# mcx/AgileRL

Measured on AMD Instinct MI355X. Metric: population env-steps/sec + learner updates/sec, 8-agent PPO at 1/2/4/8 MI355X, higher is better.
Workload: dtype f32 (GAE carry f64); 1 GPU; config 2: one 8-agent PPO population sharded 8 agents per GPU, 128 vec envs per agent, T=16, batch 128, 4 epochs, MLP enc[64]->64 + heads[64] (shared encoder), tournament every 5 iterations; population=8, pop_per_gpu=8, num_envs=128, learn_step=2048, batch_size=128, update_epochs=4, learner=fused, parallelism=population-sharded x1

## Files before the change

### agilerl_amd/csrc/learner.hip

```cpp
#include <cmath>
#include <cstdlib>
#include <type_traits>

#include "agx_common.h"
#include "rollout.h"

namespace agx {

#ifndef AGX_LEARN_UNIFORM
#define AGX_LEARN_UNIFORM 1
#endif
#ifndef AGX_LEARN_RS2
#define AGX_LEARN_RS2 0
#endif

constexpr int kNT = 512;
constexpr int kNW = kNT / kWave;
constexpr int kSB = 32;
constexpr int kMaxSlot = 10;
constexpr int kMaxK = 16;
constexpr int kMaxPT = 32;
constexpr int kMaxA = 16;
constexpr int kMaxBlk = 28;

typedef unsigned v4u __attribute__((ext_vector_type(4)));

struct NetDims {
    int D, A, ne, eo[3], ha, hc;
};

struct Blk {
    int f0, len, rowlen, l0, ldst;
};

struct LearnPlan {
    int ok;
    int D, A, ne, ein[3], eout[3], eaff[3], lat, ha, hc, H, n;
    int f_ew[3], f_eb[3], f_eg[3], f_ebe[3];
    int f_aw, f_ab, f_ag, f_abe, f_aow, f_aob, f_cw, f_cb, f_cg, f_cbe, f_cow, f_cob;
    int l_ew[3], l_eld[3], l_eb[3], l_eg[3], l_ebe[3];
    int l_hw, l_hld, l_hb, l_hg, l_hbe;
    int l_aow, l_aold, l_aob, l_cow, l_cold, l_cob;
    int param_end;
    int l_x0, ld_x0, l_xe[3], ld_xe[3], l_re[3], l_xh, ld_xh, l_rh;
    int l_s1, l_s2, ld_s;
    int l_lg, l_dlg, l_dvb, l_val, l_row;
    int l_red, red_e[3], red_h, l_stat, l_stamp;
    int l_grad;
    int lds_floats, act_floats;
    int slab;
    int nt[6], ncol[6], slot0[6], nslot[6], nslots;
    int nblk;
    Blk blk[kMaxBlk];
};

constexpr int rup(int x, int m) { return (x + m - 1) / m * m; }

constexpr LearnPlan make_plan(NetDims d) {
    LearnPlan pl{};
    pl.ok = 0;
    pl.D = d.D;
    pl.A = d.A;
    pl.ne = d.ne;
    if (pl.ne < 2 || pl.ne > 3 || pl.A < 1 || pl.A > kMaxA || pl.D < 1 || pl.D > 128) return pl;
    int prev = pl.D;
    for (int e = 0; e < pl.ne; ++e) {
        pl.ein[e] = prev;
        pl.eout[e] = d.eo[e];
        pl.eaff[e] = e < pl.ne - 1;
        if (pl.eout[e] % 16 || pl.eout[e] > 128 || pl.eout[e] < 16) return pl;
        prev = pl.eout[e];
    }
    pl.lat = prev;
    pl.ha = d.ha;
    pl.hc = d.hc;
    pl.H = pl.ha + pl.hc;
    if (pl.ha % 16 || pl.hc % 16 || pl.ha < 16 || pl.hc < 16 || pl.H > 128) return pl;
    int f = 0;
    for (int e = 0; e < pl.ne; ++e) {
        pl.f_ew[e] = f;
// ... 46 lines not shown
    pl.l_x0 = off; off += rup(kSB * pl.ld_x0, 4);
    for (int e = 0; e < pl.ne; ++e) {
        pl.ld_xe[e] = pl.eout[e] + 2;
        pl.l_xe[e] = off; off += kSB * pl.ld_xe[e];
        pl.l_re[e] = off; off += 2 * kSB;
    }
    pl.ld_xh = pl.H + 2;
    pl.l_xh = off; off += kSB * pl.ld_xh;
    pl.l_rh = off; off += 2 * kSB;
    int wmax = pl.H;
    for (int e = 0; e < pl.ne; ++e) wmax = wmax > pl.eout[e] ? wmax : pl.eout[e];
    pl.ld_s = wmax + 2;
    pl.l_s1 = off; off += kSB * pl.ld_s;
    pl.l_s2 = off; off += kSB * pl.ld_s;
    pl.l_lg = off; off += kSB * kMaxA;
    pl.l_val = off; off += kSB;
    pl.act_floats = off;
    pl.l_dlg = off; off += kSB * kMaxA;
    pl.l_dvb = off; off += kSB * kMaxA;
    pl.l_row = off; off += 6 * kSB;
    pl.l_grad = pl.l_x0;
    if (off - pl.l_x0 < pl.param_end) off = pl.l_x0 + pl.param_end;
    int red = 0;
    for (int e = 0; e < pl.ne; ++e) {
        pl.red_e[e] = red;
        red += (pl.eaff[e] ? 3 : 1) * kNW * pl.eout[e];
    }
    pl.red_h = red;
    red += 3 * kNW * pl.H;
    pl.l_red = off; off += red;
    pl.l_stat = off; off += 5 * kNW;
    off = rup(off, 2);
    pl.l_stamp = off; off += 2 * 80;
    pl.lds_floats = off;
    if (pl.lds_floats * 4 > 160 * 1024) return pl;
    pl.slab = rup(pl.param_end + 4 + 2 * kNW * kMaxK, 64);
    int slot = 0;
    for (int g = 0; g < pl.ne + 3; ++g) {
        int fo = 0, fi = 0;
        if (g < pl.ne) { fo = pl.eout[g]; fi = pl.ein[g]; }
        else if (g == pl.ne) { fo = pl.H; fi = pl.lat; }
        else if (g == pl.ne + 1) { fo = 16; fi = pl.ha + 1; }
        else { fo = 16; fi = pl.hc + 1; }
        pl.ncol[g] = (fi + 15) / 16;
        pl.nt[g] = (fo / 16) * pl.ncol[g];
        pl.slot0[g] = slot;
        pl.nslot[g] = (pl.nt[g] + kNW - 1) / kNW;
        slot += pl.nslot[g];
    }
    pl.nslots = slot;
    if (slot > kMaxSlot) return pl;
    int nb = 0;
    auto blk = [&](int f0, int len, int rowlen, int l0, int ldst) {
        if (len > 0) pl.blk[nb++] = Blk{f0, len, rowlen, l0, ldst};
    };
    for (int e = 0; e < pl.ne; ++e) {
        const int fo = pl.eout[e], fi = pl.ein[e];
        blk(pl.f_ew[e], fo * fi, fi, pl.l_ew[e], pl.l_eld[e]);
        blk(pl.f_eb[e], fo, fo, pl.l_eb[e], fo);
        if (pl.eaff[e]) {
            blk(pl.f_eg[e], fo, fo, pl.l_eg[e], fo);
            blk(pl.f_ebe[e], fo, fo, pl.l_ebe[e], fo);
        }
    }
    blk(pl.f_aw, pl.ha * pl.lat, pl.lat, pl.l_hw, pl.l_hld);
    blk(pl.f_ab, pl.ha, pl.ha, pl.l_hb, pl.ha);
// ... 499 lines not shown
            asm volatile("s_getreg_b32 %0, hwreg(HW_REG_XCC_ID)" : "=s"(x));
            __hip_atomic_store(xc + kk, (unsigned)(x & 15) + 1u, __ATOMIC_RELAXED, __HIP_MEMORY_SCOPE_AGENT);
            asm volatile("s_waitcnt vmcnt(0)" ::: "memory");
            unsigned *ctr = g.cnt + 2 * g.P + 1 + p;
            __hip_atomic_fetch_add(ctr, 1u, __ATOMIC_RELAXED, __HIP_MEMORY_SCOPE_AGENT);
            unsigned spins = 0;
            int ok = 1;
            while (__hip_atomic_load(ctr, __ATOMIC_RELAXED, __HIP_MEMORY_SCOPE_AGENT) < (unsigned)g.K) {
                __builtin_amdgcn_s_sleep(1);
                if (++spins > kSpinMax) {
                    __hip_atomic_store(tmo_v, 1u, __ATOMIC_RELAXED, __HIP_MEMORY_SCOPE_AGENT);
                    if (err_v) __hip_atomic_fetch_or(err_v, 1u, __ATOMIC_RELAXED, __HIP_MEMORY_SCOPE_AGENT);
                    ok = 0;
                    break;
                }
            }
            stat[4 * kNW] = ok ? 1.f : 0.f;
        }
        __syncthreads();
        if (stat[4 * kNW] == 0.f) return;
        const int ln = vlane();
        const unsigned v = ln < g.K ? __hip_atomic_load(xc + ln, __ATOMIC_RELAXED, __HIP_MEMORY_SCOPE_AGENT) : 0u;
        const unsigned v0 = __builtin_amdgcn_readlane(v, 0);
        bool same = v0 != 0u;
        for (int q = 1; q < g.K; ++q) same = same && __builtin_amdgcn_readlane(v, q) == v0;
        local = same && !g.write_through;
    }

    float *slab_p = in_vgpr(g.slabs + (g.K > 1 ? (size_t)p * 2 * g.K * pl.slab : 0));
    float *sum_p = in_vgpr(g.sums + (g.K > 1 ? (size_t)p * 2 * pl.slab : 0));
    unsigned *ctr1 = in_vgpr(g.cnt + p);
    unsigned *ctr2 = in_vgpr(g.cnt + g.P + 1 + p);
    unsigned *ctr3 = in_vgpr(g.cnt + 3 * g.P + 1 + (size_t)g.P * kMaxK + p);
    for (int e = 0; e < Ep; ++e) {
        for (int mb = 0; mb < nmb; ++mb) {
            const long long s0 = (long long)mb * Bp;
            const int bsz = (int)((s0 + Bp <= S) ? Bp : S - s0);
            const float inv_b = 1.f / (float)bsz;
            const int tid = vtid();
            f4 acc[kMaxSlot];
#pragma unroll
            for (int s = 0; s < kMaxSlot; ++s) acc[s] = f4{0.f, 0.f, 0.f, 0.f};
            for (int i = tid; i < pl.l_stat - pl.l_red; i += kNT) sm[pl.l_red + i] = 0.f;
            float lsum = 0.f, klsum = 0.f;
            const int upd = e * nmb + mb;
            float *base = g.K > 1 ? to_sgpr(slab_p + (size_t)(upd & 1) * g.K * pl.slab) : nullptr;
            const auto slab_rsrc = __builtin_amdgcn_make_buffer_rsrc(base + (size_t)kk * pl.slab, 0,
                                                                     __builtin_amdgcn_readfirstlane(pl.slab * 4),
                                                                     0x00020000);
            auto emit_tiles = [&](auto gc, auto fn) {
                constexpr int gg = decltype(gc)::value;
                AGX_IDS;
#pragma unroll
                for (int j = 0; j < pl.nslot[gg]; ++j) {
                    const int t = wave + kNW * j;
                    if (t < pl.nt[gg]) {
                        const int o0 = (t / pl.ncol[gg]) * 16, i0 = (t % pl.ncol[gg]) * 16;
                        const int col = i0 + lr16;
#pragma unroll
                        for (int i = 0; i < 4; ++i) {
                            const int o = o0 + lq * 4 + i;
                            const float x = acc[pl.slot0[gg] + j][i];
                            if constexpr (gg < pl.ne) {
                                if (col < pl.ein[gg]) fn(pl.l_ew[gg] + o * pl.l_eld[gg] + col, x);
                            } else if constexpr (gg == pl.ne) {
                                fn(pl.l_hw + o * pl.l_hld + col, x);
                            } else if constexpr (gg == pl.ne + 1) {
                                if (o < pl.A) {
                                    if (col < pl.ha) fn(pl.l_aow + o * pl.l_aold + col, x);
                                    else if (col == pl.ha) fn(pl.l_aob + o, x);
                                }
                            } else {
                                if (o == 0) {
                                    if (col < pl.hc) fn(pl.l_cow + col, x);
                                    else if (col == pl.hc) fn(pl.l_cob, x);
                                }
                            }
                        }
                    }
                }
            };
            auto put_l = [&](int l, float x) {
                __builtin_amdgcn_raw_buffer_store_b32(__builtin_bit_cast(unsigned, x), slab_rsrc, l * 4, 0, 0);
            };
            auto put_w = [&](int l, float x) {
                __builtin_amdgcn_raw_buffer_store_b32(__builtin_bit_cast(unsigned, x), slab_rsrc, l * 4, 0, 16);
            };
            auto slab_put = [&](int l, float x) {
                if (local) put_l(l, x);
                else put_w(l, x);
            };
            auto emit_slab = [&](auto gc) {
                if (local) emit_tiles(gc, put_l);
                else emit_tiles(gc, put_w);
            };
            const auto sum_rsrc = __builtin_amdgcn_make_buffer_rsrc(
                g.K > 1 ? to_sgpr(sum_p + (size_t)(upd & 1) * pl.slab) : nullptr, 0,
                __builtin_amdgcn_readfirstlane(pl.slab * 4), 0x00020000);
            auto partner_sync = [&](unsigned *ctr, unsigned target, int st0, int st1) -> bool {
                asm volatile("s_waitcnt vmcnt(0)" ::: "memory");
                __syncthreads();
                const int tid = vtid();
                if (tid == 0) {
                    const unsigned before = __hip_atomic_fetch_add(ctr, 1u, __ATOMIC_RELAXED, __HIP_MEMORY_SCOPE_AGENT);
                    AGX_STAMP(st0);
                    unsigned spins = 0;
                    int ok = 1;
                    while (before + 1u < target &&
                           __hip_atomic_load(ctr, __ATOMIC_RELAXED, __HIP_MEMORY_SCOPE_AGENT) < target) {
                        __builtin_amdgcn_s_sleep(1);
                        if (++spins > kSpinMax) {
                            __hip_atomic_store(tmo_v, 1u, __ATOMIC_RELAXED, __HIP_MEMORY_SCOPE_AGENT);
                            if (err_v) __hip_atomic_fetch_or(err_v, 1u, __ATOMIC_RELAXED, __HIP_MEMORY_SCOPE_AGENT);
                            ok = 0;
                            break;
                        }
                    }
                    asm volatile("s_waitcnt vmcnt(0)" ::: "memory");
                    stat[4 * kNW] = ok ? 1.f : 0.f;
                    AGX_STAMP(st1);
                }
                __syncthreads();
                return stat[4 * kNW] != 0.f;
            };
            const bool direct = g.K > 1;

            for (int sb = kk * SB; sb < bsz; sb += g.K * SB) {
                const bool last_sb = sb + g.K * SB >= bsz;
                const int nrow = bsz - sb < SB ? bsz - sb : SB;
                const int jsb = (sb / SB) / g.K;
                const int stb = jsb < 4 ? jsb * 16 : 80;
                const int tid = vtid();
                AGX_STAMP(stb + 0);
                {
                    auto commit = [&](const Pre &x) {
                        __builtin_amdgcn_s_waitcnt(0x0F70);
#pragma unroll
                        for (int k = 0; k < kPreObs; ++k) {
                            const int i = tid + k * kNT;
                            if (i < SB * pl.D) sm[pl.l_x0 + (i / pl.D) * pl.ld_x0 + i % pl.D] = i < nrow * pl.D ? x.ob[k] : 0.f;
                        }
                        constexpr int npad = pl.ld_x0 - pl.D;
#pragma unroll
                        for (int k = 0; k < (SB * npad + kNT - 1) / kNT; ++k) {
                            const int i = tid + k * kNT;
                            if (i < SB * npad) sm[pl.l_x0 + (i / npad) * pl.ld_x0 + pl.D + i % npad] = 0.f;
                        }
                        if (tid < 4 * kSB) rowf[tid] = tid % kSB < nrow ? __builtin_bit_cast(float, x.rv) : 0.f;
                        else if (tid < 5 * kSB) acts[tid - 4 * kSB] = tid - 4 * kSB < nrow ? (int)x.rv : 0;
                        else if (tid < 6 * kSB) legal[tid - 5 * kSB] = (has_mask && tid - 5 * kSB < nrow) ? x.rv : 0xffffffffu;
                    };
                    if constexpr (!kPrefetch) {
                        commit(fetch(e, mb, sb));
                    } else {
                        if (pre.e != e || pre.mb != mb || pre.sb != sb) pre = fetch(e, mb, sb);
                        commit(pre);
                        AGX_STAMP(stb + 4);
                        int ne = e, nm = mb, ns = sb + g.K * SB;
// ... 148 lines not shown
                            c2 += dxh[i] * xh[i];
                        }
                    }
                    const float rs0 = rl ? r0 : 0.f, rs1 = rl ? r1 : 0.f;
                    const float ma1 = rsum(a1) * (1.f / (float)F0), ma2 = rsum(a2) * (1.f / (float)F0);
                    const float mc1 = rsum(c1) * (1.f / (float)F1), mc2 = rsum(c2) * (1.f / (float)F1);
                    float *rd = sm + pl.l_red + pl.red_h;
                    float cs[3][NC];
#pragma unroll
                    for (int i = 0; i < NC; ++i) {
                        const int j = sub + W * i;
                        const bool g0 = W * i < split;
                        const float dz = (g0 ? rs0 : rs1) * (dxh[i] - (g0 ? ma1 : mc1) - xh[i] * (g0 ? ma2 : mc2));
                        if (rl) sm[pl.l_s2 + r * pl.ld_s + j] = dz;
                        cs[0][i] = rl ? dz : 0.f;
                        cs[1][i] = dyp[i] * xh[i];
                        cs[2][i] = dyp[i];
                    }
                    if constexpr (W == 16) {
#pragma unroll
                        for (int k = 0; k < 3; ++k)
#pragma unroll
                            for (int i = 0; i < NC; ++i) cs[k][i] += swz16(cs[k][i]);
                    }
                    if constexpr (W == 32 || (W == 16 && SB > 16)) {
#pragma unroll
                        for (int k = 0; k < 3; ++k)
#pragma unroll
                            for (int i = 0; i < NC; ++i)
                                cs[k][i] += __builtin_bit_cast(
                                    float, __builtin_amdgcn_ds_bpermute((lane ^ 32) << 2, __builtin_bit_cast(int, cs[k][i])));
                    }
                    if (lane < W) {
#pragma unroll
                        for (int k = 0; k < 3; ++k) {
                            float o[NC];
#pragma unroll
                            for (int i = 0; i < NC; ++i) o[i] = rd[(k * kNW + wave) * F + sub + W * i];
#pragma unroll
                            for (int i = 0; i < NC; ++i) rd[(k * kNW + wave) * F + sub + W * i] = o[i] + cs[k][i];
                        }
                    }
                }
                __syncthreads();
                AGX_STAMP(stb + 3);

                auto ln_bwd = [&](auto Fc, auto dybc, auto ldyc, auto xbc, auto ldxc, auto rbc, auto gbc, auto bbc,
                                  auto redc, auto affc) {
                    constexpr int F = decltype(Fc)::value;
                    constexpr int dyb = decltype(dybc)::value, ldy = decltype(ldyc)::value;
                    constexpr int xb = decltype(xbc)::value, ldx = decltype(ldxc)::value;
                    constexpr int rb = decltype(rbc)::value, gb = decltype(gbc)::value, bb = decltype(bbc)::value;
                    constexpr int red = decltype(redc)::value;
                    constexpr bool aff = decltype(affc)::value;
                    constexpr int W = (SB == 8 && F % 64 == 0) ? 64 : ((SB <= 16 && F % 32 == 0) ? 32 : 16);
                    constexpr int NC = F / W;
                    const int lane = vlane(), wave = swave();
                    const int sub = lane & (W - 1);
                    const int r = wrow<W>(lane, wave);
                    const bool rl = r < SB;
                    float xh[NC], dxh[NC], dyp[NC];
                    float a1 = 0.f, a2 = 0.f;
                    const float rs0 = rl ? sm[rb + 2 * r] : 0.f;
#pragma unroll
                    for (int i = 0; i < NC; ++i) {
                        const int j = sub + W * i;
                        const float dy = rl ? sm[dyb + r * ldy + j] : 0.f;
                        xh[i] = rl ? sm[xb + r * ldx + j] : 0.f;
                        const float gam = aff ? sm[gb + j] : 1.f;
                        const float y = aff ? xh[i] * gam + sm[bb + j] : xh[i];
                        dyp[i] = y > 0.f ? dy : 0.f;
                        dxh[i] = dyp[i] * gam;
                        a1 += dxh[i];
                        a2 += dxh[i] * xh[i];
                    }
                    const float ma1 = wrow_sum<W>(a1) * (1.f / (float)F), ma2 = wrow_sum<W>(a2) * (1.f / (float)F);
                    float *rd = sm + pl.l_red + red;
                    constexpr int NV = aff ? 3 : 1;
                    float cs[NV][NC];
#pragma unroll
                    for (int i = 0; i < NC; ++i) {
                        const int j = sub + W * i;
                        const float dz = rs0 * (dxh[i] - ma1 - xh[i] * ma2);
                        if (rl) sm[pl.l_s2 + r * pl.ld_s + j] = dz;
                        cs[0][i] = rl ? dz : 0.f;
                        if constexpr (aff) {
                            cs[1][i] = dyp[i] * xh[i];
                            cs[2][i] = dyp[i];
                        }
                    }
                    if constexpr (W == 16) {
#pragma unroll
                        for (int k = 0; k < NV; ++k)
#pragma unroll
                            for (int i = 0; i < NC; ++i)
                                cs[k][i] += __builtin_bit_cast(
                                    float, __builtin_amdgcn_ds_swizzle(__builtin_bit_cast(int, cs[k][i]), 0x401f));
                    }
                    if constexpr (W == 32 || (W == 16 && SB > 16)) {
#pragma unroll
                        for (int k = 0; k < NV; ++k)
#pragma unroll
                            for (int i = 0; i < NC; ++i)
                                cs[k][i] += __builtin_bit_cast(
                                    float, __builtin_amdgcn_ds_bpermute((lane ^ 32) << 2, __builtin_bit_cast(int, cs[k][i])));
                    }
                    if (lane < W) {
#pragma unroll
                        for (int k = 0; k < NV; ++k) {
                            float o[NC];
#pragma unroll
                            for (int i = 0; i < NC; ++i) o[i] = rd[(k * kNW + wave) * F + sub + W * i];
#pragma unroll
                            for (int i = 0; i < NC; ++i) rd[(k * kNW + wave) * F + sub + W * i] = o[i] + cs[k][i];
                        }
                    }
                };
                {
                    AGX_IDS;
                    constexpr int ga = pl.ne + 1, gc = pl.ne + 2;
#pragma unroll
                    for (int j = 0; j < pl.nslot[ga]; ++j) {
                        const int t = wave + kNW * j;
                        if (t < pl.nt[ga]) {
                            const int i0 = (t % pl.ncol[ga]) * 16;
                            acc[pl.slot0[ga] + j] = mfma_tile<SB>(
                                acc[pl.slot0[ga] + j], [&](int m, int k) { return sm[pl.l_dlg + k * kMaxA + m]; },
                                [&](int k, int n) {
                                    const int c = i0 + n;
                                    const float x = sm[pl.l_s1 + k * pl.ld_s + (c < pl.ha ? c : pl.ha - 1)];
                                    return x * (c < pl.ha ? 1.f : 0.f) + (c == pl.ha ? 1.f : 0.f);
                                });
                        }
                    }
#pragma unroll
                    for (int j = 0; j < pl.nslot[gc]; ++j) {
                        const int t = wave + kNW * j;
                        if (t < pl.nt[gc]) {
                            const int i0 = (t % pl.ncol[gc]) * 16;
                            acc[pl.slot0[gc] + j] = mfma_tile<SB>(
                                acc[pl.slot0[gc] + j], [&](int m, int k) { return sm[pl.l_dvb + k * kMaxA + m]; },
                                [&](int k, int n) {
                                    const int c = i0 + n;
                                    const float x = sm[pl.l_s1 + k * pl.ld_s + pl.ha + (c < pl.hc ? c : pl.hc - 1)];
                                    return x * (c < pl.hc ? 1.f : 0.f) + (c == pl.hc ? 1.f : 0.f);
                                });
                        }
// ... 9 lines not shown
                        if (t < pl.nt[gh]) {
                            const int o0 = (t / pl.ncol[gh]) * 16, i0 = (t % pl.ncol[gh]) * 16;
                            acc[pl.slot0[gh] + j] = mfma_tile<SB>(
                                acc[pl.slot0[gh] + j], [&](int m, int k) { return sm[pl.l_s2 + k * pl.ld_s + o0 + m]; },
                                [&](int k, int n) { return relu(sm[pl.l_xe[Le] + k * pl.ld_xe[Le] + i0 + n]); });
                        }
                    }
                    if (direct && last_sb) emit_slab(IC(gh));
                    constexpr int MT = m_tiles<SB>();
                    constexpr int nt = MT * (pl.lat / 16);
                    for (int t = wave; t < nt; t += kNW) {
                        const int m0 = (t % MT) * 16, n0 = (t / MT) * 16;
                        f4 c = f4{0.f, 0.f, 0.f, 0.f};
                        c = mfma_tile<pl.H>(c, [&](int m, int k) { return sm[pl.l_s2 + (m0 + m) * pl.ld_s + k]; },
                                            [&](int k, int n) { return sm[pl.l_hw + k * pl.l_hld + n0 + n]; });
                        if (SB >= 16 || lq * 4 < SB) {
#pragma unroll
                            for (int i = 0; i < 4; ++i) sm[pl.l_xh + (m0 + lq * 4 + i) * pl.ld_xh + n0 + lr16] = c[i];
                        }
                    }
                }
                __syncthreads();
                AGX_STAMP(stb + 6);

                auto enc_bwd = [&](auto Lc) {
                    constexpr int L = decltype(Lc)::value;
                    constexpr int fin = pl.ein[L], fout = pl.eout[L];
                    AGX_IDS;
                    constexpr int dyb = L == pl.ne - 1 ? pl.l_xh : pl.l_s1;
                    constexpr int ldy = L == pl.ne - 1 ? pl.ld_xh : pl.ld_s;
                    ln_bwd(IC(fout), IC(dyb), IC(ldy), IC(pl.l_xe[L]), IC(pl.ld_xe[L]), IC(pl.l_re[L]), IC(pl.l_eg[L]),
                           IC(pl.l_ebe[L]), IC(pl.red_e[L]), BC(pl.eaff[L] != 0));
                    __syncthreads();
                    constexpr bool in_aff = L > 0 && pl.eaff[L > 0 ? L - 1 : 0];
                    constexpr int xb = L == 0 ? pl.l_x0 : pl.l_xe[L > 0 ? L - 1 : 0];
                    constexpr int ldx = L == 0 ? pl.ld_x0 : pl.ld_xe[L > 0 ? L - 1 : 0];
                    constexpr int gbase = L > 0 ? pl.l_eg[L > 0 ? L - 1 : 0] : 0;
                    constexpr int bbase = L > 0 ? pl.l_ebe[L > 0 ? L - 1 : 0] : 0;
#pragma unroll
                    for (int j = 0; j < pl.nslot[L]; ++j) {
                        const int t = wave + kNW * j;
                        if (t < pl.nt[L]) {
                            const int o0 = (t / pl.ncol[L]) * 16, i0 = (t % pl.ncol[L]) * 16;
                            const int col = i0 + lr16;
                            const bool cv = col < fin;
                            const float gam = (in_aff && cv) ? sm[gbase + col] : 1.f;
                            const float bet = (in_aff && cv) ? sm[bbase + col] : 0.f;
                            acc[pl.slot0[L] + j] = mfma_tile<SB>(
                                acc[pl.slot0[L] + j], [&](int m, int k) { return sm[pl.l_s2 + k * pl.ld_s + o0 + m]; },
                                [&](int k, int n) {
                                    const float x = sm[xb + k * ldx + i0 + n];
                                    if constexpr (L == 0) return x;
                                    else return cv ? relu(x * gam + bet) : 0.f;
                                });
                        }
                    }
                    if (direct && last_sb) emit_slab(IC(L));
                    if constexpr (L > 0) {
                        constexpr int MT = m_tiles<SB>();
                        constexpr int nt = MT * (fin / 16);
                        for (int t = wave; t < nt; t += kNW) {
                            const int m0 = (t % MT) * 16, n0 = (t / MT) * 16;
                            f4 c = f4{0.f, 0.f, 0.f, 0.f};
                            c = mfma_tile<fout>(c, [&](int m, int k) { return sm[pl.l_s2 + (m0 + m) * pl.ld_s + k]; },
                                                [&](int k, int n) { return sm[pl.l_ew[L] + k * pl.l_eld[L] + n0 + n]; });
                            if (SB >= 16 || lq * 4 < SB) {
#pragma unroll
                                for (int i = 0; i < 4; ++i) sm[pl.l_s1 + (m0 + lq * 4 + i) * pl.ld_s + n0 + lr16] = c[i];
                            }
                        }
                    }
                    __syncthreads();
                };
                if constexpr (pl.ne == 3) enc_bwd(IC(2));
                enc_bwd(IC(1));
                enc_bwd(IC(0));
                AGX_STAMP(stb + 7);
            }

            float *G = sm + pl.l_grad;
            auto gput = [&](int l, float x) { G[l] = x; };
            if (!direct) {
                emit_tiles(IC(0), gput);
                emit_tiles(IC(1), gput);
                if constexpr (pl.ne == 3) emit_tiles(IC(2), gput);
                emit_tiles(IC(pl.ne), gput);
                emit_tiles(IC(pl.ne + 1), gput);
                emit_tiles(IC(pl.ne + 2), gput);
            } else if (kk * SB >= bsz) {
                emit_slab(IC(0));
                emit_slab(IC(1));
                if constexpr (pl.ne == 3) emit_slab(IC(2));
                emit_slab(IC(pl.ne));
                emit_slab(IC(pl.ne + 1));
                emit_slab(IC(pl.ne + 2));
            }
            auto vdump = [&](auto Lc, auto put) {
                constexpr int L = decltype(Lc)::value;
                constexpr int F = L < pl.ne ? pl.eout[L < pl.ne ? L : 0] : pl.H;
                constexpr int nv = (L < pl.ne && !pl.eaff[L < pl.ne ? L : 0]) ? 1 : 3;
                constexpr int red = L < pl.ne ? pl.red_e[L < pl.ne ? L : 0] : pl.red_h;
                const int tid = vtid();
#pragma unroll
                for (int rnd = 0; rnd < (nv * F + kNT - 1) / kNT; ++rnd) {
                    const int idx = tid + rnd * kNT;
                    if (idx >= nv * F) break;
                    const int k = idx / F, j = idx % F;
                    float pv[kNW];
#pragma unroll
                    for (int w = 0; w < kNW; ++w) pv[w] = sm[pl.l_red + red + (k * kNW + w) * F + j];
                    float x = 0.f;
#pragma unroll
                    for (int w = 0; w < kNW; ++w) x += pv[w];
                    int l;
                    if constexpr (L < pl.ne) {
                        l = (k == 0 ? pl.l_eb[L < pl.ne ? L : 0] : (k == 1 ? pl.l_eg[L < pl.ne ? L : 0] : pl.l_ebe[L < pl.ne ? L : 0])) + j;
                    } else {
                        l = (k == 0 ? pl.l_hb : (k == 1 ? pl.l_hg : pl.l_hbe)) + j;
                    }
                    put(l, x);
                }
            };
            auto vdump_all = [&](auto put) {
                vdump(IC(0), put);
                vdump(IC(1), put);
                if constexpr (pl.ne == 3) vdump(IC(2), put);
                vdump(IC(pl.ne), put);
            };
            if (!direct) vdump_all(gput);
            else if (local) vdump_all(put_l);
            else vdump_all(put_w);
            AGX_STAMP(64 + 9);
            __syncthreads();
            float lmb = lsum, klmb = klsum;
            {
                AGX_IDS;
                block_sum2(lmb, klmb, stat, 2, lane, wave);
            }
            float gr[kMaxPT];
            constexpr int NQ = (2 * kNW * KM + 63) / 64;
            float vq[NQ];
            if (g.K > 1) {
                if (tid == 0) {
                    slab_put(pl.param_end, lmb);
                    slab_put(pl.param_end + 1, klmb);
                }
                if (!partner_sync(ctr1, (unsigned)(g.K * (upd + 1)), 64 + 11, 64 + 12)) return;
                {
                    const int tid = vtid();
                    const auto rs = __builtin_amdgcn_make_buffer_rsrc(
                        base, 0, __builtin_amdgcn_readfirstlane(g.K * pl.slab * 4), 0x00020000);
                    bool rs_done = false;
#if AGX_LEARN_RS2
                    if constexpr (JN == 1) {
                        if (oc1 - oc0 <= kNT / 2) {
                            constexpr int KH = KM / 2;
                            const int h = tid >= kNT / 2 ? 1 : 0;
                            const int c = oc0 + (tid & (kNT / 2 - 1));
                            const int cl = c < oc1 ? c : oc0;
                            f4 x[KH];
#pragma unroll
                            for (int q = 0; q < KH; ++q) {
                                const int qq = KH * h + q, qs = qq < g.K ? qq : g.K - 1;
                                const f4 v = __builtin_bit_cast(
                                    f4, __builtin_amdgcn_raw_buffer_load_b128(rs, (qs * pl.slab + 4 * cl) * 4, 0, 16));
                                x[q] = qq < g.K ? v : f4{0.f, 0.f, 0.f, 0.f};
                            }
                            f4 t = x[0];
#pragma unroll
                            for (int q = 1; q < KH; ++q) t += x[q];
                            f4 *xch = reinterpret_cast<f4 *>(sm + pl.l_x0);
                            if (h) xch[tid - kNT / 2] = t;
                            __syncthreads();
                            if (!h) {
                                t += xch[tid];
                                if (c == n4) {
                                    if (local) __builtin_amdgcn_raw_buffer_store_b128(__builtin_bit_cast(v4u, t), sum_rsrc, c * 16, 0, 0);
                                    else __builtin_amdgcn_raw_buffer_store_b128(__builtin_bit_cast(v4u, t), sum_rsrc, c * 16, 0, 16);
                                }
                            }
#pragma unroll
                            for (int cc = 0; cc < 4; ++cc) gr[cc] = (!h && c < pc1) ? t[cc] : 0.f;
                            rs_done = true;
                        }
                    }
#endif
#pragma unroll
                    for (int j = 0; j < kUsed4; ++j) {
                        if (rs_done) break;
                        const int c = oc0 + tid + kNT * j;
                        f4 t = f4{0.f, 0.f, 0.f, 0.f};
                        if (j >= jn_own) {
#pragma unroll
                            for (int cc = 0; cc < 4; ++cc) gr[4 * j + cc] = 0.f;
                            continue;
                        }
                        if (c < oc1) {
                            f4 x[KM];
#pragma unroll
                            for (int q = 0; q < KM; ++q)
                                x[q] = q < g.K ? __builtin_bit_cast(f4, __builtin_amdgcn_raw_buffer_load_b128(
                                                                           rs, (q * pl.slab + 4 * c) * 4, 0, 16))
                                               : f4{0.f, 0.f, 0.f, 0.f};
                            t = x[0];
#pragma unroll
                            for (int q = 1; q < KM; ++q)
                                if (q < g.K) t += x[q];
                            if (c == n4) {
                                if (local) __builtin_amdgcn_raw_buffer_store_b128(__builtin_bit_cast(v4u, t), sum_rsrc, c * 16, 0, 0);
                                else __builtin_amdgcn_raw_buffer_store_b128(__builtin_bit_cast(v4u, t), sum_rsrc, c * 16, 0, 16);
                            }
                        }
#pragma unroll
                        for (int cc = 0; cc < 4; ++cc) gr[4 * j + cc] = c < pc1 ? t[cc] : 0.f;
                    }
                    AGX_STAMP(64 + 3);
                    float n0 = 0.f, n1 = 0.f;
#pragma unroll
                    for (int i = 0; i < 4 * kUsed4; ++i) {
                        if ((i >> 2) >= jn_own) break;
                        const bool valid = (vbits >> i) & 1u, crit = (gbits >> i) & 1u;
                        gr[i] = valid ? gr[i] : 0.f;
                        const float x2 = gr[i] * gr[i];
                        n1 += crit ? x2 : 0.f;
                        n0 += crit ? 0.f : x2;
                    }
                    const int lane = vlane(), wave = swave();
                    const float r0 = row_sum(n0), r1 = row_sum(n1);
                    const float w0 = readlane_f(r0, 0) + readlane_f(r0, 16) + readlane_f(r0, 32) + readlane_f(r0, 48);
                    const float w1 = readlane_f(r1, 0) + readlane_f(r1, 16) + readlane_f(r1, 32) + readlane_f(r1, 48);
                    if (lane < 2) {
                        const float w = lane ? w1 : w0;
                        const int o = (pl.param_end + 4 + (kk * kNW + wave) * 2 + lane) * 4;
                        if (local) __builtin_amdgcn_raw_buffer_store_b32(__builtin_bit_cast(unsigned, w), sum_rsrc, o, 0, 0);
                        else __builtin_amdgcn_raw_buffer_store_b32(__builtin_bit_cast(unsigned, w), sum_rsrc, o, 0, 16);
                    }
                }
                AGX_STAMP(64 + 13);
                if (!partner_sync(ctr2, (unsigned)(g.K * (upd + 1)), 64 + 8, 64 + 15)) return;
                {
                    const int lane = vlane();
                    const int np = 2 * kNW * g.K;
#pragma unroll
                    for (int q = 0; q < NQ; ++q) {
                        const float x = __builtin_bit_cast(
                            float, __builtin_amdgcn_raw_buffer_load_b32(sum_rsrc, (pl.param_end + 4 + 64 * q + lane) * 4, 0, 16));
                        vq[q] = lane + 64 * q < np ? x : 0.f;
                    }
                }
                const unsigned lw = __builtin_amdgcn_raw_buffer_load_b32(sum_rsrc, pl.param_end * 4, 0, 16);
                const unsigned kw = __builtin_amdgcn_raw_buffer_load_b32(sum_rsrc, (pl.param_end + 1) * 4, 0, 16);
                lmb = __builtin_bit_cast(float, __builtin_amdgcn_readfirstlane(lw));
                klmb = __builtin_bit_cast(float, __builtin_amdgcn_readfirstlane(kw));
            }

            float t0 = 0.f, t1 = 0.f;
            if (!direct) {
                const f4 *G4 = reinterpret_cast<const f4 *>(G);
#pragma unroll
                for (int j = 0; j < kUsed4; ++j) {
                    const int c = own_c(j);
                    const f4 x = c < pc1 ? G4[c] : f4{0.f, 0.f, 0.f, 0.f};
#pragma unroll
                    for (int cc = 0; cc < 4; ++cc) gr[4 * j + cc] = x[cc];
                }
                float n0 = 0.f, n1 = 0.f;
#pragma unroll
                for (int i = 0; i < 4 * kUsed4; ++i) {
                    const bool valid = (vbits >> i) & 1u, crit = (gbits >> i) & 1u;
                    gr[i] = valid ? gr[i] : 0.f;
                    const float x2 = gr[i] * gr[i];
                    n1 += crit ? x2 : 0.f;
                    n0 += crit ? 0.f : x2;
                }
                AGX_IDS;
                {
                    const float r0 = row_sum(n0), r1 = row_sum(n1);
                    const float w0 = readlane_f(r0, 0) + readlane_f(r0, 16) + readlane_f(r0, 32) + readlane_f(r0, 48);
                    const float w1 = readlane_f(r1, 0) + readlane_f(r1, 16) + readlane_f(r1, 32) + readlane_f(r1, 48);
                    if (lane == 0) {
                        stat[wave] = w0;
                        stat[kNW + wave] = w1;
                    }
                }
                __syncthreads();
                for (int i = 0; i < kNW; ++i) {
// ... 125 lines not shown
        const int l = 4 * own_c(i >> 2) + (i & 3);
        if ((vbits >> i) & 1u) {
            int grp;
            const int f = lds_to_flat<C>(l, grp);
            gp[f] = sm[l];
            gm[f] = am[i];
            gv[f] = av[i];
        }
    }
    if constexpr (ST)
        if (g.stamps && b == 0 && tid < 80) g.stamps[tid] = reinterpret_cast<const long long *>(sm + pl.l_stamp)[tid];
    if (tid == 0 && kk == 0) {
        if (loss_out_v) loss_out_v[p] = loss_total / ((float)S * (float)Ep);
        if (kl_out_v) kl_out_v[p] = n_done ? (float)(kl_total / (double)n_done) : 0.f;
        if (epochs_out_v) epochs_out_v[p] = epochs_done;
        *step_v = step0 + n_done;
    }
#undef IC
#undef BC
}

__global__ void ppo_gather_kernel(const float *__restrict__ obs, const long long *__restrict__ act,
                                  const float *__restrict__ old_logp, const float *__restrict__ adv,
                                  const float *__restrict__ ret, const float *__restrict__ old_v,
                                  const double *__restrict__ adv_stats, const long long *__restrict__ perms,
                                  const unsigned char *__restrict__ masks, int A,
                                  long long S, int D, int P, float *__restrict__ gobs, int *__restrict__ gact,
                                  unsigned *__restrict__ gmask, float *__restrict__ grow,
                                  unsigned *__restrict__ counters, int ncounters, const int *__restrict__ epochs_p,
                                  unsigned *__restrict__ err) {
    const int ep = blockIdx.y;
    const int p = ep % P;
    const long long j = (long long)blockIdx.x * blockDim.x + threadIdx.x;
    if (blockIdx.x == 0 && blockIdx.y == 0)
        for (int i = threadIdx.x; i < ncounters; i += blockDim.x) counters[i] = 0u;
    if (j >= S) return;
    if (epochs_p && ep / P >= epochs_p[p]) return;
    long long src = perms[(size_t)ep * S + j];
    if (src < 0 || src >= S) {
        if (err) __hip_atomic_fetch_or(err, AGX_LEARN_ERR_PERM, __ATOMIC_RELAXED, __HIP_MEMORY_SCOPE_AGENT);
        src = 0;
    }
    const size_t sp = (size_t)p * S + src;
    for (int d = 0; d < D; ++d) gobs[((size_t)ep * S + j) * D + d] = obs[sp * D + d];
    gact[(size_t)ep * S + j] = (int)act[sp];
    if (masks) {
        unsigned bits = 0;
        for (int a = 0; a < A; ++a) bits |= (masks[sp * A + a] != 0 ? 1u : 0u) << a;
        gmask[(size_t)ep * S + j] = bits;
    }
    float *gr = grow + (size_t)ep * 4 * S;
    double a = adv[sp];
    if (adv_stats) a = (a - adv_stats[2 * p]) * (1.0 / (adv_stats[2 * p + 1] + 1e-8));
    gr[j] = old_logp[sp];
    gr[S + j] = (float)a;
    gr[2 * S + j] = ret[sp];
    gr[3 * S + j] = old_v[sp];
}

template <class C>
__device__ __forceinline__ void act_body(const ActArgs &g, float *sm, bool resident, long long *st = nullptr) {
    constexpr LearnPlan pl = C::plan;
    const int p = blockIdx.y, n0 = blockIdx.x * kSB;
    const int tid = threadIdx.x, lane = tid & 63, wave = tid >> 6;
    const int nrow = g.N - n0 < kSB ? g.N - n0 : kSB;
    const float *ob = g.obs + (size_t)p * g.obs_pstride + (size_t)n0 * pl.D;
    constexpr int kObsIt = (kSB * pl.D + kNT - 1) / kNT;
    float obv[kObsIt];
// ... 246 lines not shown
    return (size_t)L.plan->lds_floats * sizeof(float);
}

static int max_partners(int64_t P) {
    int k = kMaxK;
    if (const char *e = getenv("AGX_LEARN_SPLIT")) k = atoi(e);
    if (k < 1) k = 1;
    if (k > kMaxK) k = kMaxK;
    const int64_t fit = cu_count() / (P > 0 ? P : 1);
    if (fit < k) k = fit < 1 ? 1 : (int)fit;
    return k;
}
static void pick_split(int64_t P, int64_t batch, int &K, int &SB) {
    const int kmax = max_partners(P);
    int sb = kmax >= 16 ? 8 : (kmax >= 8 ? 16 : 32);
    if (const char *e = getenv("AGX_LEARN_SB")) {
        const int v = atoi(e);
        if (v == 8 || v == 16 || v == 32) sb = v;
    }
    const int64_t nsb = (batch + sb - 1) / sb;
    K = sb == 32 ? (kmax > 4 ? 4 : kmax) : (sb == 16 ? (kmax > 8 ? 8 : kmax) : kmax);
    if (K > nsb) K = (int)nsb;
    if (K < 1) K = 1;
    SB = sb;
}
struct LearnWs {
    size_t cnt, gobs, gact, gmask, grow, slabs, sums, total;
};
static LearnWs learn_ws(const LearnPlan &pl, int64_t P, int64_t S, int64_t epochs) {
    LearnWs w;
    const size_t per = (size_t)epochs * P * S;
    auto up = [](size_t x) { return (x + 255) & ~(size_t)255; };
    w.cnt = 0;
    w.gobs = up(((size_t)(4 + kMaxK) * P + 1) * 4);
    w.gact = w.gobs + up(per * pl.D * 4);
    w.gmask = w.gact + up(per * 4);
    w.grow = w.gmask + up(per * 4);
    w.slabs = w.grow + up(per * 4 * 4);
    const int64_t fit = cu_count() / (P > 0 ? P : 1);
    const int K = fit < 1 ? 1 : (fit > kMaxK ? kMaxK : (int)fit);
    w.sums = w.slabs + (K > 1 ? up((size_t)P * 2 * K * pl.slab * 4) : 0);
    w.total = w.sums + (K > 1 ? (size_t)P * 2 * pl.slab * 4 : 0);
    return w;
}

extern "C" size_t agx_ppo_learn_workspace_bytes(const agx_ppo_net *net, int64_t P, int64_t S, int64_t epochs) {
    Launcher L;
    if (!find_launcher(net, L) || P <= 0 || S <= 0 || epochs <= 0) return 0;
    return learn_ws(*L.plan, P, S, epochs).total;
}

extern "C" int agx_debug_learn_stamps(int64_t *buf) {
    static_assert(sizeof(long long) == sizeof(int64_t), "");
    g_stamps_ptr() = reinterpret_cast<long long *>(buf);
    return AGX_OK;
}

extern "C" int agx_debug_rollout_stamps(int64_t *buf) {
    g_roll_stamps_ptr() = reinterpret_cast<long long *>(buf);
    return AGX_OK;
}

extern "C" int agx_ppo_learn_prepare(const agx_ppo_net *net, void *workspace, void *stream) {
    (void)workspace;
    (void)stream;
    AGX_REQUIRE(net, "agx_ppo_learn_prepare: null pointer");
    Launcher L;
// ... 212 lines not shown
```

Measured before the change: 10.24 million env-steps/s.

## Replace second partner barrier with tagged 64-bit mailbox words and early bias dumps

Replaces the second counter-based partner_sync in the multi-CU learner with per-update tagged 64-bit atomic words. Each partner writes its loss and row partials with the update index in the high half, and readers spin until every tag matches, so there is no separate barrier round-trip. It also dumps the LayerNorm and bias reductions into the slab early, right after each layer's backward on the last sub-batch, instead of at the end. It skips zeroing the reduction buffers when a CTA processes only one sub-batch, and clears the counters in parallel across the whole gather grid. The cost is a larger workspace and more complex memory-ordering assumptions, since relaxed atomics with workgroup scope are used for local stores.

```diff
diff --git a/agilerl_amd/csrc/learner.hip b/agilerl_amd/csrc/learner.hip
--- a/agilerl_amd/csrc/learner.hip
+++ b/agilerl_amd/csrc/learner.hip
@@ -12,6 +12,18 @@
 #endif
 #ifndef AGX_LEARN_RS2
 #define AGX_LEARN_RS2 0
+#endif
+#ifndef AGX_LEARN_B2_TAGGED
+#define AGX_LEARN_B2_TAGGED 1
+#endif
+#ifndef AGX_LEARN_B2_SWEEP1
+#define AGX_LEARN_B2_SWEEP1 1
+#endif
+#ifndef AGX_LEARN_VEC_EARLY
+#define AGX_LEARN_VEC_EARLY 1
+#endif
+#ifndef AGX_LEARN_STORE1
+#define AGX_LEARN_STORE1 1
 #endif
 
 constexpr int kNT = 512;
@@ -22,6 +34,10 @@
 constexpr int kMaxPT = 32;
 constexpr int kMaxA = 16;
 constexpr int kMaxBlk = 28;
+
+constexpr int kB2Words = 2 * kNW * kMaxK + 2;
+constexpr size_t b2_words_off(size_t P) { return ((4 + kMaxK) * P + 1 + 3) / 4 * 4; }
+typedef __attribute__((address_space(1))) unsigned long long gu64;
 
 typedef unsigned v4u __attribute__((ext_vector_type(4)));
 
@@ -45,7 +61,7 @@
     int l_x0, ld_x0, l_xe[3], ld_xe[3], l_re[3], l_xh, ld_xh, l_rh;
     int l_s1, l_s2, ld_s;
     int l_lg, l_dlg, l_dvb, l_val, l_row;
-    int l_red, red_e[3], red_h, l_stat, l_stamp;
+    int l_red, red_e[3], red_h, l_stat, l_stamp, l_b2x;
     int l_grad;
     int lds_floats, act_floats;
     int slab;
@@ -158,6 +174,7 @@
     pl.l_stat = off; off += 5 * kNW;
     off = rup(off, 2);
     pl.l_stamp = off; off += 2 * 80;
+    pl.l_b2x = off; off += 2 * kNW * kMaxK + 4;
     pl.lds_floats = off;
     if (pl.lds_floats * 4 > 160 * 1024) return pl;
     pl.slab = rup(pl.param_end + 4 + 2 * kNW * kMaxK, 64);
@@ -723,6 +740,11 @@
     unsigned *ctr1 = in_vgpr(g.cnt + p);
     unsigned *ctr2 = in_vgpr(g.cnt + g.P + 1 + p);
     unsigned *ctr3 = in_vgpr(g.cnt + 3 * g.P + 1 + (size_t)g.P * kMaxK + p);
+#if AGX_LEARN_B2_TAGGED
+    unsigned long long *b2_p =
+        in_vgpr(reinterpret_cast<unsigned long long *>(g.cnt + b2_words_off(g.P)) + (size_t)p * 2 * kB2Words);
+    (void)ctr2;
+#endif
     for (int e = 0; e < Ep; ++e) {
         for (int mb = 0; mb < nmb; ++mb) {
             const long long s0 = (long long)mb * Bp;
@@ -732,7 +754,9 @@
             f4 acc[kMaxSlot];
 #pragma unroll
             for (int s = 0; s < kMaxSlot; ++s) acc[s] = f4{0.f, 0.f, 0.f, 0.f};
-            for (int i = tid; i < pl.l_stat - pl.l_red; i += kNT) sm[pl.l_red + i] = 0.f;
+            const bool single = AGX_LEARN_STORE1 && kk * SB < bsz && kk * SB + g.K * SB >= bsz;
+            if (!single)
+                for (int i = tid; i < pl.l_stat - pl.l_red; i += kNT) sm[pl.l_red + i] = 0.f;
             float lsum = 0.f, klsum = 0.f;
             const int upd = e * nmb + mb;
             float *base = g.K > 1 ? to_sgpr(slab_p + (size_t)(upd & 1) * g.K * pl.slab) : nullptr;
@@ -785,9 +809,40 @@
                 if (local) emit_tiles(gc, put_l);
                 else emit_tiles(gc, put_w);
             };
+            auto vdump = [&](auto Lc, auto put) {
+                constexpr int L = decltype(Lc)::value;
+                constexpr int F = L < pl.ne ? pl.eout[L < pl.ne ? L : 0] : pl.H;
+                constexpr int nv = (L < pl.ne && !pl.eaff[L < pl.ne ? L : 0]) ? 1 : 3;
+                constexpr int red = L < pl.ne ? pl.red_e[L < pl.ne ? L : 0] : pl.red_h;
+                const int tid = vtid();
+#pragma unroll
+                for (int rnd = 0; rnd < (nv * F + kNT - 1) / kNT; ++rnd) {
+                    const int idx = tid + rnd * kNT;
+                    if (idx >= nv * F) break;
+                    const int k = idx / F, j = idx % F;
+                    float pv[kNW];
+#pragma unroll
+                    for (int w = 0; w < kNW; ++w) pv[w] = sm[pl.l_red + red + (k * kNW + w) * F + j];
+                    float x = 0.f;
+#pragma unroll
+                    for (int w = 0; w < kNW; ++w) x += pv[w];
+                    int l;
+                    if constexpr (L < pl.ne) {
+                        l = (k == 0 ? pl.l_eb[L < pl.ne ? L : 0] : (k == 1 ? pl.l_eg[L < pl.ne ? L : 0] : pl.l_ebe[L < pl.ne ? L : 0])) + j;
+                    } else {
+                        l = (k == 0 ? pl.l_hb : (k == 1 ? pl.l_hg : pl.l_hbe)) + j;
+                    }
+                    put(l, x);
+                }
+            };
+            auto vdump_slab = [&](auto Lc) {
+                if (local) vdump(Lc, put_l);
+                else vdump(Lc, put_w);
+            };
             const auto sum_rsrc = __builtin_amdgcn_make_buffer_rsrc(
                 g.K > 1 ? to_sgpr(sum_p + (size_t)(upd & 1) * pl.slab) : nullptr, 0,
                 __builtin_amdgcn_readfirstlane(pl.slab * 4), 0x00020000);
+            (void)sum_rsrc;
             auto partner_sync = [&](unsigned *ctr, unsigned target, int st0, int st1) -> bool {
                 asm volatile("s_waitcnt vmcnt(0)" ::: "memory");
                 __syncthreads();
@@ -815,6 +870,7 @@
                 return stat[4 * kNW] != 0.f;
             };
             const bool direct = g.K > 1;
+            const bool vec_early = AGX_LEARN_VEC_EARLY && direct;
 
             for (int sb = kk * SB; sb < bsz; sb += g.K * SB) {
                 const bool last_sb = sb + g.K * SB >= bsz;
@@ -1029,18 +1085,26 @@
                                     float, __builtin_amdgcn_ds_bpermute((lane ^ 32) << 2, __builtin_bit_cast(int, cs[k][i])));
                     }
                     if (lane < W) {
-#pragma unroll
-                        for (int k = 0; k < 3; ++k) {
-                            float o[NC];
-#pragma unroll
-                            for (int i = 0; i < NC; ++i) o[i] = rd[(k * kNW + wave) * F + sub + W * i];
-#pragma unroll
-                            for (int i = 0; i < NC; ++i) rd[(k * kNW + wave) * F + sub + W * i] = o[i] + cs[k][i];
+                        if (single) {
+#pragma unroll
+                            for (int k = 0; k < 3; ++k)
+#pragma unroll
+                                for (int i = 0; i < NC; ++i) rd[(k * kNW + wave) * F + sub + W * i] = cs[k][i] + 0.f;
+                        } else {
+#pragma unroll
+                            for (int k = 0; k < 3; ++k) {
+                                float o[NC];
+#pragma unroll
+                                for (int i = 0; i < NC; ++i) o[i] = rd[(k * kNW + wave) * F + sub + W * i];
+#pragma unroll
+                                for (int i = 0; i < NC; ++i) rd[(k * kNW + wave) * F + sub + W * i] = o[i] + cs[k][i];
+                            }
                         }
                     }
                 }
                 __syncthreads();
                 AGX_STAMP(stb + 3);
+                if (vec_early && last_sb) vdump_slab(IC(pl.ne));
 
                 auto ln_bwd = [&](auto Fc, auto dybc, auto ldyc, auto xbc, auto ldxc, auto rbc, auto gbc, auto bbc,
                                   auto redc, auto affc) {
@@ -1103,13 +1167,20 @@
                                     float, __builtin_amdgcn_ds_bpermute((lane ^ 32) << 2, __builtin_bit_cast(int, cs[k][i])));
                     }
                     if (lane < W) {
-#pragma unroll
-                        for (int k = 0; k < NV; ++k) {
-                            float o[NC];
-#pragma unroll
-                            for (int i = 0; i < NC; ++i) o[i] = rd[(k * kNW + wave) * F + sub + W * i];
-#pragma unroll
-                            for (int i = 0; i < NC; ++i) rd[(k * kNW + wave) * F + sub + W * i] = o[i] + cs[k][i];
+                        if (single) {
+#pragma unroll
+                            for (int k = 0; k < NV; ++k)
+#pragma unroll
+                                for (int i = 0; i < NC; ++i) rd[(k * kNW + wave) * F + sub + W * i] = cs[k][i] + 0.f;
+                        } else {
+#pragma unroll
+                            for (int k = 0; k < NV; ++k) {
+                                float o[NC];
+#pragma unroll
+                                for (int i = 0; i < NC; ++i) o[i] = rd[(k * kNW + wave) * F + sub + W * i];
+#pragma unroll
+                                for (int i = 0; i < NC; ++i) rd[(k * kNW + wave) * F + sub + W * i] = o[i] + cs[k][i];
+                            }
                         }
                     }
                 };
@@ -1185,6 +1256,7 @@
                     ln_bwd(IC(fout), IC(dyb), IC(ldy), IC(pl.l_xe[L]), IC(pl.ld_xe[L]), IC(pl.l_re[L]), IC(pl.l_eg[L]),
                            IC(pl.l_ebe[L]), IC(pl.red_e[L]), BC(pl.eaff[L] != 0));
                     __syncthreads();
+                    if (vec_early && last_sb) vdump_slab(Lc);
                     constexpr bool in_aff = L > 0 && pl.eaff[L > 0 ? L - 1 : 0];
                     constexpr int xb = L == 0 ? pl.l_x0 : pl.l_xe[L > 0 ? L - 1 : 0];
                     constexpr int ldx = L == 0 ? pl.ld_x0 : pl.ld_xe[L > 0 ? L - 1 : 0];
@@ -1248,32 +1320,6 @@
                 emit_slab(IC(pl.ne + 1));
                 emit_slab(IC(pl.ne + 2));
             }
-            auto vdump = [&](auto Lc, auto put) {
-                constexpr int L = decltype(Lc)::value;
-                constexpr int F = L < pl.ne ? pl.eout[L < pl.ne ? L : 0] : pl.H;
-                constexpr int nv = (L < pl.ne && !pl.eaff[L < pl.ne ? L : 0]) ? 1 : 3;
-                constexpr int red = L < pl.ne ? pl.red_e[L < pl.ne ? L : 0] : pl.red_h;
-                const int tid = vtid();
-#pragma unroll
-                for (int rnd = 0; rnd < (nv * F + kNT - 1) / kNT; ++rnd) {
-                    const int idx = tid + rnd * kNT;
-                    if (idx >= nv * F) break;
-                    const int k = idx / F, j = idx % F;
-                    float pv[kNW];
-#pragma unroll
-                    for (int w = 0; w < kNW; ++w) pv[w] = sm[pl.l_red + red + (k * kNW + w) * F + j];
-                    float x = 0.f;
-#pragma unroll
-                    for (int w = 0; w < kNW; ++w) x += pv[w];
-                    int l;
-                    if constexpr (L < pl.ne) {
-                        l = (k == 0 ? pl.l_eb[L < pl.ne ? L : 0] : (k == 1 ? pl.l_eg[L < pl.ne ? L : 0] : pl.l_ebe[L < pl.ne ? L : 0])) + j;
-                    } else {
-                        l = (k == 0 ? pl.l_hb : (k == 1 ? pl.l_hg : pl.l_hbe)) + j;
-                    }
-                    put(l, x);
-                }
-            };
             auto vdump_all = [&](auto put) {
                 vdump(IC(0), put);
                 vdump(IC(1), put);
@@ -1281,8 +1327,10 @@
                 vdump(IC(pl.ne), put);
             };
             if (!direct) vdump_all(gput);
-            else if (local) vdump_all(put_l);
-            else vdump_all(put_w);
+            else if (!vec_early || kk * SB >= bsz) {
+                if (local) vdump_all(put_l);
+                else vdump_all(put_w);
+            }
             AGX_STAMP(64 + 9);
             __syncthreads();
             float lmb = lsum, klmb = klsum;
@@ -1299,6 +1347,24 @@
                     slab_put(pl.param_end + 1, klmb);
                 }
                 if (!partner_sync(ctr1, (unsigned)(g.K * (upd + 1)), 64 + 11, 64 + 12)) return;
+#if AGX_LEARN_B2_TAGGED
+                gu64 *const b2w = (gu64 *)(b2_p + (size_t)(upd & 1) * kB2Words);
+                const unsigned long long b2tag = (unsigned long long)(unsigned)(upd + 1) << 32;
+                auto b2_store = [&](gu64 *w, unsigned v) {
+                    if (local) __hip_atomic_store(w, b2tag | v, __ATOMIC_RELAXED, __HIP_MEMORY_SCOPE_WORKGROUP);
+                    else __hip_atomic_store(w, b2tag | v, __ATOMIC_RELAXED, __HIP_MEMORY_SCOPE_AGENT);
+                };
+                auto put_loss = [&](f4 t) {
+                    const float lw = t[0], kw = t[1];
+                    b2_store(b2w + 2 * kNW * kMaxK, __builtin_bit_cast(unsigned, lw));
+                    b2_store(b2w + 2 * kNW * kMaxK + 1, __builtin_bit_cast(unsigned, kw));
+                };
+#else
+                auto put_loss = [&](f4 t) {
+                    if (local) __builtin_amdgcn_raw_buffer_store_b128(__builtin_bit_cast(v4u, t), sum_rsrc, n4 * 16, 0, 0);
+                    else __builtin_amdgcn_raw_buffer_store_b128(__builtin_bit_cast(v4u, t), sum_rsrc, n4 * 16, 0, 16);
+                };
+#endif
                 {
                     const int tid = vtid();
                     const auto rs = __builtin_amdgcn_make_buffer_rsrc(
@@ -1327,10 +1393,7 @@
                             __syncthreads();
                             if (!h) {
                                 t += xch[tid];
-                                if (c == n4) {
-                                    if (local) __builtin_amdgcn_raw_buffer_store_b128(__builtin_bit_cast(v4u, t), sum_rsrc, c * 16, 0, 0);
-                                    else __builtin_amdgcn_raw_buffer_store_b128(__builtin_bit_cast(v4u, t), sum_rsrc, c * 16, 0, 16);
-                                }
+                                if (c == n4) put_loss(t);
                             }
 #pragma unroll
                             for (int cc = 0; cc < 4; ++cc) gr[cc] = (!h && c < pc1) ? t[cc] : 0.f;
@@ -1359,10 +1422,7 @@
 #pragma unroll
                             for (int q = 1; q < KM; ++q)
                                 if (q < g.K) t += x[q];
-                            if (c == n4) {
-                                if (local) __builtin_amdgcn_raw_buffer_store_b128(__builtin_bit_cast(v4u, t), sum_rsrc, c * 16, 0, 0);
-                                else __builtin_amdgcn_raw_buffer_store_b128(__builtin_bit_cast(v4u, t), sum_rsrc, c * 16, 0, 16);
-                            }
+                            if (c == n4) put_loss(t);
                         }
 #pragma unroll
                         for (int cc = 0; cc < 4; ++cc) gr[4 * j + cc] = c < pc1 ? t[cc] : 0.f;
@@ -1382,13 +1442,77 @@
                     const float r0 = row_sum(n0), r1 = row_sum(n1);
                     const float w0 = readlane_f(r0, 0) + readlane_f(r0, 16) + readlane_f(r0, 32) + readlane_f(r0, 48);
                     const float w1 = readlane_f(r1, 0) + readlane_f(r1, 16) + readlane_f(r1, 32) + readlane_f(r1, 48);
+#if AGX_LEARN_B2_TAGGED
+                    AGX_STAMP(64 + 13);
+                    if (lane < 2)
+                        b2_store(b2w + (kk * kNW + wave) * 2 + lane, __builtin_bit_cast(unsigned, lane ? w1 : w0));
+                    AGX_STAMP(64 + 8);
+#else
                     if (lane < 2) {
                         const float w = lane ? w1 : w0;
                         const int o = (pl.param_end + 4 + (kk * kNW + wave) * 2 + lane) * 4;
                         if (local) __builtin_amdgcn_raw_buffer_store_b32(__builtin_bit_cast(unsigned, w), sum_rsrc, o, 0, 0);
                         else __builtin_amdgcn_raw_buffer_store_b32(__builtin_bit_cast(unsigned, w), sum_rsrc, o, 0, 16);
                     }
+#endif
                 }
+#if AGX_LEARN_B2_TAGGED
+                {
+                    const int lane = vlane();
+                    const int np = 2 * kNW * g.K;
+                    const unsigned tag = (unsigned)(upd + 1);
+                    unsigned lo[NQ], ll = 0u;
+#if AGX_LEARN_B2_SWEEP1
+                    unsigned *b2x = reinterpret_cast<unsigned *>(sm + pl.l_b2x);
+                    bool swept = true;
+                    if (swave() == 0) {
+#endif
+                    for (unsigned spins = 0;;) {
+                        unsigned long long x[NQ];
+#pragma unroll
+                        for (int q = 0; q < NQ; ++q)
+                            x[q] = __hip_atomic_load(b2w + 64 * q + lane, __ATOMIC_RELAXED, __HIP_MEMORY_SCOPE_AGENT);
+                        const unsigned long long xl =
+                            __hip_atomic_load(b2w + 2 * kNW * kMaxK + (lane & 1), __ATOMIC_RELAXED, __HIP_MEMORY_SCOPE_AGENT);
+                        unsigned bad = (unsigned)(xl >> 32) ^ tag;
+                        ll = (unsigned)xl;
+#pragma unroll
+                        for (int q = 0; q < NQ; ++q) {
+                            bad |= lane + 64 * q < np ? (unsigned)(x[q] >> 32) ^ tag : 0u;
+                            lo[q] = (unsigned)x[q];
+                        }
+                        if (__all(bad == 0u)) break;
+                        __builtin_amdgcn_s_sleep(1);
+                        if (++spins > kSpinMax) {
+                            __hip_atomic_store(tmo_v, 1u, __ATOMIC_RELAXED, __HIP_MEMORY_SCOPE_AGENT);
+                            if (err_v) __hip_atomic_fetch_or(err_v, AGX_LEARN_ERR_TIMEOUT, __ATOMIC_RELAXED, __HIP_MEMORY_SCOPE_AGENT);
+#if AGX_LEARN_B2_SWEEP1
+                            swept = false;
+                            break;
+#else
+                            return;
+#endif
+                        }
+                    }
+#if AGX_LEARN_B2_SWEEP1
+#pragma unroll
+                        for (int q = 0; q < NQ; ++q) b2x[lane + 64 * q] = lo[q];
+                        if (lane < 2) b2x[2 * kNW * kMaxK + lane] = ll;
+                        if (lane == 0) stat[4 * kNW] = swept ? 1.f : 0.f;
+                    }
+                    __syncthreads();
+                    if (stat[4 * kNW] == 0.f) return;
+#pragma unroll
+                    for (int q = 0; q < NQ; ++q) lo[q] = b2x[lane + 64 * q];
+                    ll = b2x[2 * kNW * kMaxK + (lane & 1)];
+#endif
+#pragma unroll
+                    for (int q = 0; q < NQ; ++q) vq[q] = lane + 64 * q < np ? __builtin_bit_cast(float, lo[q]) : 0.f;
+                    lmb = __builtin_bit_cast(float, __builtin_amdgcn_readlane(ll, 0));
+                    klmb = __builtin_bit_cast(float, __builtin_amdgcn_readlane(ll, 1));
+                }
+                AGX_STAMP(64 + 15);
+#else
                 AGX_STAMP(64 + 13);
                 if (!partner_sync(ctr2, (unsigned)(g.K * (upd + 1)), 64 + 8, 64 + 15)) return;
                 {
@@ -1405,6 +1529,7 @@
                 const unsigned kw = __builtin_amdgcn_raw_buffer_load_b32(sum_rsrc, (pl.param_end + 1) * 4, 0, 16);
                 lmb = __builtin_bit_cast(float, __builtin_amdgcn_readfirstlane(lw));
                 klmb = __builtin_bit_cast(float, __builtin_amdgcn_readfirstlane(kw));
+#endif
             }
 
             float t0 = 0.f, t1 = 0.f;
@@ -1596,8 +1721,9 @@
     const int ep = blockIdx.y;
     const int p = ep % P;
     const long long j = (long long)blockIdx.x * blockDim.x + threadIdx.x;
-    if (blockIdx.x == 0 && blockIdx.y == 0)
-        for (int i = threadIdx.x; i < ncounters; i += blockDim.x) counters[i] = 0u;
+    if (blockIdx.y == 0)
+        for (int i = blockIdx.x * blockDim.x + threadIdx.x; i < ncounters; i += gridDim.x * blockDim.x)
+            counters[i] = 0u;
     if (j >= S) return;
     if (epochs_p && ep / P >= epochs_p[p]) return;
     long long src = perms[(size_t)ep * S + j];
@@ -1910,7 +2036,7 @@
     const size_t per = (size_t)epochs * P * S;
     auto up = [](size_t x) { return (x + 255) & ~(size_t)255; };
     w.cnt = 0;
-    w.gobs = up(((size_t)(4 + kMaxK) * P + 1) * 4);
+    w.gobs = up(b2_words_off((size_t)P) * 4 + (AGX_LEARN_B2_TAGGED ? (size_t)P * 2 * kB2Words * 8 : 0));
     w.gact = w.gobs + up(per * pl.D * 4);
     w.gmask = w.gact + up(per * 4);
     w.grow = w.gmask + up(per * 4);
```

Result: faster. 10.86 million env-steps/s, median of 6 (+6.1%).
